# vvvwo/KSS-ICP

Hardware: AMD Instinct MI355X
Metric: icp_iterations_per_sec (higher is better)
Workload: dtype f32; 1 GPU; C2: one 100000x100000 uniform-sphere pair per GPU, 50 fixed ICP iterations + fitness pass per step (exact NN + cov reduce + host 3x3 SVD), R_z(10deg), jitter 1e-3; n_src=100000, n_tgt=100000, pairs_per_gpu=1, nn_engine=cell list + brute-force fallback, nn_arithmetic=reference (no fma)

## Files before the change

### kss-icp_amd/csrc/kss_engine.hip

```cpp
#pragma clang fp contract(off)

#include <emmintrin.h>
#include <limits>

#include "kss_ctx.hpp"
#include "kss_pair_device.hpp"

namespace kss {

static int restore_zero_at_rest(kss_ctx* c);

static int resident_rows_limit(kss_ctx* c) {
    if (c->cu_count <= 0) {
        hipDeviceProp_t prop;
        c->cu_count = hipGetDeviceProperties(&prop, c->device) == hipSuccess && prop.multiProcessorCount > 0 ? prop.multiProcessorCount : 1;
        (void)hipGetLastError();
    }
    return c->cu_count;
}

constexpr int PUB_PAIRS = 32;
static int ensure_pub(kss_ctx* c, int npairs = PUB_PAIRS);

struct PairGeom {
// ... 516 lines not shown
        hipDeviceProp_t prop;
        void* bar = nullptr;
        if (want_bar && hipGetDeviceProperties(&prop, c->device) == hipSuccess && prop.isLargeBar &&
            hipExtMallocWithFlags(&bar, 4096, hipDeviceMallocFinegrained) == hipSuccess && bar) {
            if (hipMemset(bar, 0, 4096) == hipSuccess && hipDeviceSynchronize() == hipSuccess) {
                c->gate_bar = (unsigned int*)bar;
                c->gated.supported = 1;
                return true;
            }
            hipFree(bar);
        }
        (void)hipGetLastError();
        void *x = nullptr, *xd = nullptr;
        if (ensure(c, c->g_gate, 256) == KSS_OK && hipMemsetAsync(c->g_gate.p, 0, 256, c->stream) == hipSuccess &&
            hipHostMalloc(&x, 2 * sizeof(PairState), hipHostMallocMapped) == hipSuccess && hipHostGetDevicePointer(&xd, x, 0) == hipSuccess) {
            std::memset(x, 0, 2 * sizeof(PairState));
            c->h_xf = (PairState*)x; c->h_xf_dev = (PairState*)xd;
            c->gated.supported = 1;
        } else {
            (void)hipGetLastError();
            if (x) hipHostFree(x);
        }
    }
    return c->gated.supported == 1;
}

static void gated_release(kss_ctx* c, const PairState& st, int skip) {
    if (c->gate_bar) {
        int words[16];
        std::memcpy(words, &st, sizeof st);
        words[14] = skip;
        unsigned int* slot = c->gate_bar + 32 * c->gated.slot;
        static const long torn_at = getenv("KSS_TEST_TORN_GATE") ? atol(getenv("KSS_TEST_TORN_GATE")) : -1;
        static long released = 0;
        const bool torn = ++released == torn_at;
        for (int pass = torn ? 0 : 1; pass < 2; ++pass) {
            for (int g = 0; g < 5; ++g) {
                const unsigned tag = (unsigned)c->gated.stamp + kss_mix3((unsigned)words[3 * g], (unsigned)words[3 * g + 1], (unsigned)words[3 * g + 2]);
                const int w1 = pass == 0 && g == 1 ? words[3 * g + 1] ^ 0x00010000 : words[3 * g + 1];
                const __m128i v = _mm_set_epi32((int)tag, words[3 * g + 2], w1, words[3 * g]);
                _mm_store_si128((__m128i*)(slot + 4 * g), v);
            }
            _mm_sfence();
            if (pass == 0) {
                const auto t0 = std::chrono::steady_clock::now();
                while (std::chrono::duration<double, std::micro>(std::chrono::steady_clock::now() - t0).count() < 200.0) __builtin_ia32_pause();
            }
        }
    } else {
        PairState* rec = &c->h_xf[c->gated.slot];
        for (int k = 0; k < 12; ++k) rec->m[k] = st.m[k];
        rec->active = st.active; rec->apply = st.apply; rec->pad[0] = skip;
        __atomic_store_n(&rec->pad[1], c->gated.stamp, __ATOMIC_RELEASE);
    }
    kss_ctx::Gated& G = c->gated;
    if (!skip && --G.steps_left > 0) {
        G.slot ^= 1;
        G.stamp += 1;
        G.seq += 1;
        const void* in = G.d_out; G.d_out = const_cast<void*>(G.d_in); G.d_in = in;
    } else {
        G.pending = false;
        G.steps_left = 0;
    }
}

static void gated_cancel(kss_ctx* c) {
    if (!c->gated.pending) return;
    PairState none;
    std::memset(&none, 0, sizeof none);
    gated_release(c, none, 1);
}

struct GatedGuard {
    kss_ctx* c;
    explicit GatedGuard(kss_ctx* c_) : c(c_) {}
    ~GatedGuard() { gated_cancel(c); c->gated.want_next = false; }
};

static float skin_setting() {
    static const float skin = getenv("KSS_SKIN") ? (float)atof(getenv("KSS_SKIN")) : 0.25f;
    return skin;
}
static int gate_polls_setting() {
    static const int gate_polls = getenv("KSS_GATE_POLLS") ? atoi(getenv("KSS_GATE_POLLS")) : (1 << 22);
    return gate_polls;
}

static PassArgs pass_args(kss_ctx* c, const IcpPlan& pl, const float4* d_in, float4* d_out, double max_d2,
                          int32_t* d_idx_out, float* d_d2_out) {
    PassArgs a;
    std::memset(&a, 0, sizeof a);
    a.src_in = d_in; a.src_out = d_out;
    a.cell_start = (const int32_t*)c->g_start.p + 1;
    a.sorted = (const float4*)c->g_sorted.p;
    a.tgt4 = (const float4*)c->tgt4.p;
    a.nn_win = (float4*)c->g_pos.p;
    a.nn_state = (float2*)c->g_nnst.p;
    a.skin = skin_setting();
    a.chain_len = 1;
    a.gate_polls = gate_polls_setting();
    a.chained = d_in != (const float4*)c->src0.p ? 1 : c->fit_last ? 2 : 0;
    a.src_last0 = (const float4*)c->cur[0].p; a.src_last1 = (const float4*)c->cur[1].p;
    a.keys = (unsigned long long*)c->keys.p;
    a.list = (int32_t*)c->g_list.p; a.list_count = (int32_t*)c->g_count.p;
    a.total_rows = pl.total_rows;
    a.use_prev = c->nn_have ? 1 : 0;
    a.max_d2 = max_d2;
    a.rows = (Granule*)c->partials.p;
    a.pub = c->h_seq_dev;
    a.idx_out = d_idx_out; a.d2_out = d_d2_out;
    {
        static const long torn_at = getenv("KSS_TEST_TORN_SLOT") ? atol(getenv("KSS_TEST_TORN_SLOT")) : -1;
        static long launches = 0;
        a.test_torn = torn_at > 0 && ++launches == torn_at ? 1 : 0;
    }
    if (pl.gridb) {
        a.pairs = (const GridPairDev*)c->g_pairs.p;
        a.row_pair = (const int32_t*)c->g_rowpair.p;
        a.defer_pairs = pl.npairs > resident_rows_limit(c) ? pl.npairs : 0;
    } else {
        a.pair0 = pl.gpairs[0];
    }
    return a;
}

struct GridPass {
    const IcpPlan& pl;
    bool fma, full;
    const float4* d_in; float4* d_out;
    double max_d2;
    int32_t* d_idx_out; float* d_d2_out;
    PassArgs a;
    int nblk;
    unsigned long long* stamps2 = nullptr;
    bool plain_args = false;
    unsigned long long want_seq = 0;
    bool via_gate = false;
};

static void grid_launch_plain(kss_ctx* c, GridPass& g) {
    ProfScope ps(c, KSS_K_GRID_NN);
    g.a.ps0 = ((const PairState*)c->h_state)[0];
    g.a.seq = ++c->seq;
    if (g.stamps2) g.a.stamps = g.stamps2 + (size_t)(g.a.seq & 1) * g.nblk * 16;
    launch_grid_pass(c->stream, g.fma, g.full, false, true, g.a);
    c->nn_have = true;
    g.want_seq = c->seq;
}

static void grid_release_or_launch(kss_ctx* c, GridPass& g) {
    kss_ctx::Gated& G = c->gated;
    if (G.pending && G.d_in == (const void*)g.d_in && G.d_out == (void*)g.d_out && G.fma == g.fma && G.full == g.full && G.max_d2 == g.max_d2 && g.plain_args) {
        g.want_seq = G.seq;
        c->seq = std::max(c->seq, G.seq);
        if (G.chain && c->prof > 0) c->prof_n[KSS_K_GRID_CHAIN_PASS] += 1;
        g.via_gate = true;
        static const long drop_at = getenv("KSS_TEST_DROP_GATE") ? atol(getenv("KSS_TEST_DROP_GATE")) : -1;
        static long releases = 0;
        if (++releases == drop_at) { G.pending = false; G.steps_left = 0; }
        else gated_release(c, ((const PairState*)c->h_state)[0], 0);
    } else {
        gated_cancel(c);
        grid_launch_plain(c, g);
    }
}

static void grid_enqueue_next(kss_ctx* c, const GridPass& g) {
    kss_ctx::Gated& G = c->gated;
    const bool next_sampled = c->prof == 1 || (c->prof > 1 && c->prof_tick[KSS_K_GRID_NN] % (unsigned)c->prof == 0);
    static const bool want_chain = getenv("KSS_CHAIN") == nullptr || atoi(getenv("KSS_CHAIN")) != 0;
    int len = 1;
    if (G.want_next && !G.pending && g.plain_args && gated_available(c) && want_chain && c->gate_bar &&
        (g.pl.total_rows <= resident_rows_limit(c) || g.pl.total_rows == 1))
        len = std::max(1, std::min(G.max_steps, 1 << 16));
    if (!(G.want_next && !G.pending && g.plain_args && gated_available(c) && (len > 1 || !next_sampled))) return;
    if (c->prof > 1 && len == 1) ++c->prof_tick[KSS_K_GRID_NN];
    float4* nxt_out = g.d_out == (float4*)c->cur[0].p ? (float4*)c->cur[1].p : (float4*)c->cur[0].p;
    G.slot ^= 1;
    G.stamp = (G.stamp + 1) & 0x7fffffff;
    if (G.stamp == 0 || G.stamp > 0x7fffffff - len - 1) G.stamp = 1;
    PassArgs n = pass_args(c, g.pl, g.d_out, nxt_out, g.max_d2, nullptr, nullptr);
// ... 1505 lines not shown
```

### kss-icp_amd/csrc/kss_grid.hip

```cpp
#pragma clang fp contract(off)

#include <hip/hip_runtime.h>

#include <cstring>

#include <rocprim/rocprim.hpp>

#include <cstdlib>

#include "kss_internal.hpp"
#include "kss_device.hpp"

namespace kss {

__global__ __launch_bounds__(256) void grid_count2_kernel(const float4* __restrict__ tgt, int nt, int nbt, const float4* __restrict__ src, int ns,
                                                          GridParams gp, int32_t* __restrict__ counts, int32_t* __restrict__ slot) {
    const bool is_src = (int)blockIdx.x >= nbt;
    const int i = ((int)blockIdx.x - (is_src ? nbt : 0)) * 256 + (int)threadIdx.x;
    if (i >= (is_src ? ns : nt)) return;
    const float4 p = is_src ? src[i] : tgt[i];
    const int cx = cell_coord(p.x, gp.ox, gp.inv_h, gp.gx), cy = cell_coord(p.y, gp.oy, gp.inv_h, gp.gy),
              cz = cell_coord(p.z, gp.oz, gp.inv_h, gp.gz);
    slot[(is_src ? nt : 0) + i] = atomicAdd(&counts[(is_src ? gp.gx * gp.gy * gp.gz : 0) + (cz * gp.gy + cy) * gp.gx + cx], 1);
}
// ... 537 lines not shown
                    const int x0 = max(cx - r, 0), x1 = min(cx + r, gp.gx - 1);
                    for (int t = 0; t < wd * wd; ++t) {
                        const int dz = t / wd - r, dy = t % wd - r;
                        const int z = cz + dz, y = cy + dy;
                        if (z < 0 || z >= gp.gz || y < 0 || y >= gp.gy) continue;
                        const int row = (z * gp.gy + y) * gp.gx;
                        if (dz == -r || dz == r || dy == -r || dy == r) {
                            scan_range<FMA>(sorted, cs[row + x0], cs[row + x1 + 1], wx, wy, wz, wkey, wpos);
                        } else {
                            if (cx - r >= 0) scan_range<FMA>(sorted, cs[row + cx - r], cs[row + cx - r + 1], wx, wy, wz, wkey, wpos);
                            if (cx + r < gp.gx) scan_range<FMA>(sorted, cs[row + cx + r], cs[row + cx + r + 1], wx, wy, wz, wkey, wpos);
                        }
                    }
                }
                const float best = __uint_as_float((unsigned)(wkey >> 32));
                float b = __builtin_inff();
                if (cx - r > 0) b = fminf(b, wx - (gp.ox + (float)(cx - r) * gp.h));
                if (cx + r < gp.gx - 1) b = fminf(b, (gp.ox + (float)(cx + r + 1) * gp.h) - wx);
                if (cy - r > 0) b = fminf(b, wy - (gp.oy + (float)(cy - r) * gp.h));
                if (cy + r < gp.gy - 1) b = fminf(b, (gp.oy + (float)(cy + r + 1) * gp.h) - wy);
                if (cz - r > 0) b = fminf(b, wz - (gp.oz + (float)(cz - r) * gp.h));
                if (cz + r < gp.gz - 1) b = fminf(b, (gp.oz + (float)(cz + r + 1) * gp.h) - wz);
                const float bs = b - gp.eps;
                if (b == __builtin_inff()) done = true;
                else if (bs > 0.f && best < bs * bs * 0.999999f) { done = true; face2 = bs * bs; }
                if (done) { rfin = r; break; }
            }
            if (done && rfin == 1 && wkey != ~0ull)
                bnew = fminf(__builtin_amdgcn_sqrtf(fminf(fminf(m2, wrho), face2) * 0.99999f) * 0.999999f, 1e30f);
        }
        if constexpr (BATCH) {
            if (__builtin_amdgcn_ballot_w64(!done) != 0ull) {
                const float4* __restrict__ tp = a.tgt4 + pr.tgt_base;
                for (int j = 0; j < pr.tgt_n; ++j) {
                    const float4 q = tp[j];
                    const float dx = wx - q.x, dy = wy - q.y, dz = wz - q.z;
                    float d;
                    if constexpr (FMA) d = __builtin_fmaf(dx, dx, __builtin_fmaf(dy, dy, dz * dz));
                    else d = (dx * dx + dy * dy) + dz * dz;
                    const unsigned long long kk = ((unsigned long long)__float_as_uint(d) << 32) | (unsigned long long)(unsigned)j;
                    if (!done && kk < wkey) { wkey = kk; wpos = -1; }
                }
                wfell = !done;
                done = true;
            }
        }
        if (wk && sub == 0) {
            bool whave = false;
            float4 ww = make_float4(0.f, 0.f, 0.f, 0.f);
            const int io = pr.src_base + (w - pr.row_base) * PASS_BS + owner;
            if (done) {
                whave = wkey != ~0ull;
                if (whave) ww = wpos >= 0 ? sorted[wpos] : wpos == -2 ? a.nn_win[io] : a.tgt4[pr.tgt_base + (int)(unsigned)(wkey & 0xffffffffull)];
            } else {
                a.keys[io] = ~0ull;
                const int ls = atomicAdd(a.list_count, 1);
                a.list[ls] = io;
                wfell = true;
            }
            a.nn_win[io] = make_float4(ww.x, ww.y, ww.z, __uint_as_float(whave ? (unsigned)wkey : ~0u));
            a.nn_state[io] = make_float2(wfell ? 0.f : bnew, 0.f);
            s_ent[WK_X][owner] = __float_as_uint(ww.x); s_ent[WK_Y][owner] = __float_as_uint(ww.y); s_ent[WK_Z][owner] = __float_as_uint(ww.z);
            s_ent[WK_IDX][owner] = (unsigned)wkey; s_ent[WK_D2][owner] = (unsigned)(wkey >> 32);
            s_ent[WK_FL][owner] = (whave ? 1u : 0u) | (wfell ? 2u : 0u);
            s_ent[WK_R][owner] = __float_as_uint(wfell ? 0.f : bnew);
        }
        KSS_STAMP(8);
        if (a.stamps) {
            int evs = evl, mx = evl;
#pragma unroll
            for (int m = 32; m > 0; m >>= 1) { evs += __shfl_xor(evs, m, 64); mx = max(mx, __shfl_xor(mx, m, 64)); }
            if (lane == 0) {
                atomicAdd(&a.stamps[(size_t)blockIdx.x * 16 + 10], (unsigned long long)evs);
                atomicAdd(&a.stamps[(size_t)blockIdx.x * 16 + 11], (unsigned long long)(((mx + 7) / 8) * 8 * 64));
            }
        }
    }
#undef KSS_STAMP
}

#ifndef KSS_SINGLE_WAVES
#define KSS_SINGLE_WAVES 1
#endif
template <bool FMA, bool FULL, bool SEARCH, bool CHAIN, bool FIRST = false>
__global__ __launch_bounds__(PASS_BS, KSS_SINGLE_WAVES) void grid_pass_kernel(const PassArgs a) {
    static_assert(!CHAIN || SEARCH, "chained launches: search passes");
    static_assert(!FIRST || (SEARCH && !CHAIN), "the first pass: a plain search launch");
#define KSS_STAMP(k) do { if (a.stamps && threadIdx.x == 0) a.stamps[(size_t)blockIdx.x * 16 + (k)] = __builtin_amdgcn_s_memrealtime(); } while (0)
    KSS_STAMP(0);
    constexpr int BS = PASS_BS;
    const int per_xcd = (int)gridDim.x / 8;
    const int w = ((int)blockIdx.x % 8) * per_xcd + (int)blockIdx.x / 8;
    if (w >= a.total_rows) return;
    const GridPairDev pr = a.pair0;
    PairState ps = a.ps0;
    const GridParams& gp = pr.gp;
    const int32_t* __restrict__ cs = a.cell_start + pr.cell_base;
    const float4* __restrict__ sorted = a.sorted;
    constexpr int WQ = FIRST ? BS : 256;
    __shared__ int2 rowq[9][WQ];
    __shared__ double shw[BS / 64][NSUMS];
    __shared__ int s_last;
    __shared__ int sh_ps[16];
    __shared__ int s_nwalk;
    __shared__ unsigned s_ent[7][BS];
    __shared__ unsigned short s_wl[BS];
    enum { WK_X, WK_Y, WK_Z, WK_IDX, WK_D2, WK_R, WK_POS, WK_FL = WK_POS, WK_COLS };
    static_assert(sizeof(PairState) == 64, "the gated launch reads the transform record as 16 dwords");
    double (*shf)[NSUMS] = reinterpret_cast<double (*)[NSUMS]>(&rowq[0][0]);
    static_assert(sizeof(double) * PASS_FG * NSUMS <= sizeof(int2) * 9 * WQ, "shf must fit inside rowq");

    const int local = (w - pr.row_base) * BS + (int)threadIdx.x;
    const bool valid = local < pr.src_n;
    const int i = pr.src_base + local;
    const int lane = threadIdx.x & 63, wave = threadIdx.x >> 6;
    bool have = false, fell_back = false;
    float qx = 0.f, qy = 0.f, qz = 0.f, d2 = 0.f;
    float4 win = make_float4(0.f, 0.f, 0.f, 0.f);
    float4 p = make_float4(0.f, 0.f, 0.f, 0.f), prevp = make_float4(0.f, 0.f, 0.f, __uint_as_float(~0u));
    float2 st = make_float2(0.f, 0.f);
    if (valid) {
        p = SEARCH ? a.src_in[i] : a.src_out[i];
        if (!SEARCH || a.use_prev) { prevp = a.nn_win[i]; st = a.nn_state[i]; }
    }
    for (int step = 0;; ++step) {
    const bool last_step = !CHAIN || step + 1 >= a.chain_len;
    const unsigned long long seq_k = a.seq + (unsigned long long)step;
    const int gate_k = a.gate_seq != 0 ? a.gate_seq + step : 0;
    unsigned int* const gate_ptr = a.gate_dev + 32 * ((a.gate_slot + step) & 1);
    float4* const src_out_k = (step & 1) ? a.src_alt : a.src_out;
    const bool last_known = a.chained == 2 && ps.pad[0] > 0;
    const bool chained_k = step > 0 || a.chained == 1 || last_known;
    const bool has_prev = __float_as_uint(prevp.w) != ~0u;
    if constexpr (SEARCH) {
        __syncthreads();
        if (threadIdx.x == 0) s_nwalk = 0;
        __syncthreads();
    }
    KSS_STAMP(13);
    if constexpr (SEARCH) {
        if (gate_k != 0) {
            typedef unsigned int u32x4 __attribute__((ext_vector_type(4)));
            if (a.state && w == 0 && threadIdx.x < 16) {
                const int* w32 = reinterpret_cast<const int*>(a.state);
                int v = 0, n = 0;
                bool ok = true;
                for (;;) {
                    v = __hip_atomic_load(w32 + threadIdx.x, __ATOMIC_RELAXED, __HIP_MEMORY_SCOPE_SYSTEM);
                    if (__shfl(v, 15, 64) == gate_k) break;
                    __builtin_amdgcn_s_sleep(1);
                    if (++n > a.gate_polls / 2) { ok = false; break; }
                }
                if (ok) {
                    const int g = threadIdx.x;
                    const int w0 = __shfl(v, min(3 * g, 15), 64), w1 = __shfl(v, min(3 * g + 1, 15), 64), w2 = __shfl(v, min(3 * g + 2, 15), 64);
                    if (g < 5) {
                        u32x4 o;
                        o.x = (unsigned)w0; o.y = (unsigned)w1; o.z = (unsigned)w2; o.w = (unsigned)gate_k + kss_mix3(o.x, o.y, o.z);
                        unsigned int* dst = gate_ptr + 4 * g;
                        asm volatile("global_store_dwordx4 %0, %1, off sc1" ::"v"(dst), "v"(o) : "memory");
                    }
                }
            }
            if (threadIdx.x < 8) {
                const unsigned int* src = gate_ptr + 4 * min((int)threadIdx.x, 4);
                u32x4 v;
                int n = 0;
                bool ok = true;
                for (;;) {
                    asm volatile("global_load_dwordx4 %0, %1, off sc0 sc1\n\ts_waitcnt vmcnt(0)" : "=&v"(v) : "v"(src) : "memory");
                    if (__builtin_amdgcn_ballot_w64(v.w - kss_mix3(v.x, v.y, v.z) == (unsigned)gate_k) == 0xffull) break;
                    __builtin_amdgcn_s_sleep(1);
                    if (++n > a.gate_polls) { ok = false; break; }
                }
                if (threadIdx.x < 5) { sh_ps[3 * threadIdx.x] = (int)v.x; sh_ps[3 * threadIdx.x + 1] = (int)v.y; sh_ps[3 * threadIdx.x + 2] = (int)v.z; }
                if (threadIdx.x == 0) { sh_ps[15] = gate_k; s_last = ok ? 1 : 0; }
            }
            __syncthreads();
            if (!s_last) return;
            int* d32 = reinterpret_cast<int*>(&ps);
#pragma unroll
            for (int k = 0; k < 16; ++k) d32[k] = sh_ps[k];
            if (ps.pad[0] != 0) return;
            __syncthreads();
            KSS_STAMP(9);
        }
    }
    unsigned long long key = ~0ull;
    float pold_x = p.x, pold_y = p.y, pold_z = p.z;
    if (SEARCH && last_known && valid) {
        const float4 pl = (ps.pad[0] == 1 ? a.src_last0 : a.src_last1)[i];
        pold_x = pl.x; pold_y = pl.y; pold_z = pl.z;
    }
    if (valid) {
        if constexpr (SEARCH) {
            if (ps.apply) {
                const float x = p.x, y = p.y, z = p.z;
                p.x = ((ps.m[0] * x + ps.m[1] * y) + ps.m[2] * z) + ps.m[3];
                p.y = ((ps.m[4] * x + ps.m[5] * y) + ps.m[6] * z) + ps.m[7];
                p.z = ((ps.m[8] * x + ps.m[9] * y) + ps.m[10] * z) + ps.m[11];
            }
            src_out_k[i] = p;
        }
        qx = p.x; qy = p.y; qz = p.z;
        const bool qok = (qx - qx) == 0.f && (qy - qy) == 0.f && (qz - qz) == 0.f;
        if constexpr (!SEARCH) {
            if (has_prev) {
                win = prevp;
                key = point_key<FMA>(win, qx, qy, qz);
            } else if (qok) {
                key = a.keys[i];
                if (key != ~0ull) win = a.tgt4[pr.tgt_base + (int)(unsigned)(key & 0xffffffffull)];
            }
            have = key != ~0ull;
        }
    }
    if constexpr (SEARCH) {
        bool walker = false;
        float acc_keep = 0.f;
        {
            const bool qok = valid && (qx - qx) == 0.f && (qy - qy) == 0.f && (qz - qz) == 0.f;
            const SkipOut so = skip_test<FMA>(qok, qx, qy, qz, pold_x, pold_y, pold_z, prevp, st, chained_k, a.skin, gp.h);
            walker = so.walker;
            key = so.key;
            acc_keep = so.acc;
            unsigned fl = 0u;
            if (qok && !walker) {
                fl = 1u;
                a.nn_state[i] = make_float2(st.x, so.acc);
            } else if (valid && !qok) {
                a.nn_win[i] = make_float4(0.f, 0.f, 0.f, __uint_as_float(~0u));
                a.nn_state[i] = make_float2(0.f, 0.f);
            }
            const float4 c4 = walker ? make_float4(qx, qy, qz, 0.f) : prevp;
            s_ent[WK_X][threadIdx.x] = __float_as_uint(c4.x); s_ent[WK_Y][threadIdx.x] = __float_as_uint(c4.y); s_ent[WK_Z][threadIdx.x] = __float_as_uint(c4.z);
            s_ent[WK_IDX][threadIdx.x] = (unsigned)key; s_ent[WK_D2][threadIdx.x] = (unsigned)(key >> 32);
            s_ent[WK_POS][threadIdx.x] = walker ? (unsigned)so.kpos : fl;
            s_ent[WK_R][threadIdx.x] = __float_as_uint(so.rho);
        }
        const unsigned long long wm = __builtin_amdgcn_ballot_w64(walker);
        if (wm != 0ull) {
            int base = 0;
            if (lane == 0) base = atomicAdd(&s_nwalk, (int)__builtin_popcountll(wm));
            base = __builtin_amdgcn_readfirstlane(base);
            if (walker) s_wl[base + (int)__builtin_amdgcn_mbcnt_hi((unsigned)(wm >> 32), __builtin_amdgcn_mbcnt_lo((unsigned)wm, 0u))] = (unsigned short)threadIdx.x;
        }
        KSS_STAMP(14);
        __syncthreads();
        const int nwalk = s_nwalk;
        if (a.stamps && threadIdx.x == 0) a.stamps[(size_t)blockIdx.x * 16 + 12] = (unsigned long long)nwalk;
        serve_walkers<FMA, false, WQ, BS, 8, FIRST>(a, pr, cs, sorted, w, nwalk, rowq, s_ent, s_wl);
        KSS_STAMP(15);
        __syncthreads();
        {
            const unsigned fl = s_ent[WK_FL][threadIdx.x];
            have = (fl & 1u) != 0u; fell_back = (fl & 2u) != 0u;
            win = make_float4(__uint_as_float(s_ent[WK_X][threadIdx.x]), __uint_as_float(s_ent[WK_Y][threadIdx.x]), __uint_as_float(s_ent[WK_Z][threadIdx.x]), 0.f);
            key = ((unsigned long long)s_ent[WK_D2][threadIdx.x] << 32) | (unsigned long long)s_ent[WK_IDX][threadIdx.x];
            if (CHAIN && !last_step) {
                if (walker) {
                    prevp = make_float4(win.x, win.y, win.z, __uint_as_float(have ? (unsigned)key : ~0u));
                    st = make_float2(__uint_as_float(s_ent[WK_R][threadIdx.x]), 0.f);
                } else if (have) {
                    st.y = acc_keep;
                } else {
                    prevp.w = __uint_as_float(~0u);
                    st = make_float2(0.f, 0.f);
                }
            }
        }
    }
    if (valid && have) {
        d2 = __uint_as_float((unsigned)(key >> 32));
        const int oi = __float_as_int(p.w);
        if (a.idx_out) a.idx_out[oi] = (int)(unsigned)(key & 0xffffffffull);
        if (a.d2_out) a.d2_out[oi] = d2;
    }
    KSS_STAMP(1);

    const double d2d = have ? (double)d2 : 0.0;
    const bool kept = have && !(d2d > a.max_d2);
    wave_row<FULL>(have, kept, fell_back, qx, qy, qz, win, d2d, shw[wave]);
    __syncthreads();
    double r = 0.0;
    if (threadIdx.x < NSUMS)
#pragma unroll
        for (int ww = 0; ww < BS / 64; ++ww) r += shw[ww][threadIdx.x];
    KSS_STAMP(2);

    double v = 0.0 + r;
    if (pr.n_rows > 1) {
        Granule* const rows = a.rows + (int64_t)pr.row_base * NSUMS;
        if (threadIdx.x < NSUMS) row_put(rows + (int64_t)(w - pr.row_base) * NSUMS, threadIdx.x, r, seq_k);
        KSS_STAMP(3);
        if (w != pr.row_base || a.defer_pairs) {
            if (last_step) return;
            continue;
        }
        if (!rows_total<PASS_FG>(rows, pr.n_rows, seq_k, 1 << 20, shf, &s_last, v)) return;
    }
    if (threadIdx.x < NSUMS) {
        if (!FULL && (threadIdx.x == 17 || threadIdx.x == 18)) v = 0.0;
        const int64_t slot = threadIdx.x;
        if (a.test_torn && threadIdx.x == 5) {
            pub_put(a.pub, slot, v, seq_k, 0x00100000u);
            asm volatile("s_waitcnt vmcnt(0)" ::: "memory");
            for (int k = 0; k < 400; ++k) __builtin_amdgcn_s_sleep(64);
        }
        pub_put(a.pub, slot, v, seq_k);
        KSS_STAMP(4);
    }
    if (last_step) break;
    }
#undef KSS_STAMP
}

#ifndef KSS_BATCH2_WAVES
#define KSS_BATCH2_WAVES 5
#endif
template <bool FMA, bool FULL, int WQ>
__global__ __launch_bounds__(256, KSS_BATCH2_WAVES) void gridb_pass_kernel(const PassArgs a) {
#define KSS_STAMP(k) do { if (a.stamps && threadIdx.x == 0) a.stamps[(size_t)blockIdx.x * 16 + (k)] = __builtin_amdgcn_s_memrealtime(); } while (0)
    KSS_STAMP(0);
    constexpr int BS = PASS_BS, NT = 256, SPL = BS / NT;
    static_assert(SPL == 2 && WQ <= NT, "two sources per lane");
    const int per_xcd = (int)gridDim.x / 8;
    const int w = ((int)blockIdx.x % 8) * per_xcd + (int)blockIdx.x / 8;
    if (w >= a.total_rows) return;
    const int pi = a.row_pair[w];
    const GridPairDev pr = a.pairs[pi];
    const PairState ps = a.state[pi];
    if (!ps.active) return;
    const GridParams& gp = pr.gp;
    const int32_t* __restrict__ cs = a.cell_start + pr.cell_base;
    const float4* __restrict__ sorted = a.sorted;
    __shared__ int2 rowq[9][WQ];
    __shared__ double shw[BS / 64][NSUMS];
    __shared__ int s_last;
    __shared__ int s_nwalk;
    __shared__ unsigned s_ent[7][BS];
    __shared__ unsigned short s_wl[BS];
    enum { WK_X, WK_Y, WK_Z, WK_IDX, WK_D2, WK_R, WK_POS, WK_FL = WK_POS, WK_COLS };
    constexpr int SHF_ROWS = (int)(sizeof(int2) * 9 * WQ / (sizeof(double) * NSUMS));
    static_assert(SHF_ROWS >= PASS_FG, "shf must fit inside rowq");
    double (*shf)[NSUMS] = reinterpret_cast<double (*)[NSUMS]>(&rowq[0][0]);
    const int lane = threadIdx.x & 63, wave = threadIdx.x >> 6;

    bool valid[SPL];
    int idx[SPL];
    float4 p[SPL], prevp[SPL];
    float2 st[SPL];
#pragma unroll
    for (int k = 0; k < SPL; ++k) {
        const int slot = k * NT + (int)threadIdx.x;
        const int local = (w - pr.row_base) * BS + slot;
        valid[k] = local < pr.src_n;
        idx[k] = pr.src_base + local;
        p[k] = make_float4(0.f, 0.f, 0.f, 0.f);
        prevp[k] = make_float4(0.f, 0.f, 0.f, __uint_as_float(~0u));
        st[k] = make_float2(0.f, 0.f);
        if (valid[k]) {
            p[k] = a.src_in[idx[k]];
            if (a.use_prev) { prevp[k] = a.nn_win[idx[k]]; st[k] = a.nn_state[idx[k]]; }
        }
    }
    if (threadIdx.x == 0) s_nwalk = 0;
    __syncthreads();
    KSS_STAMP(13);
    const bool last_known = a.chained == 2 && ps.pad[0] > 0;
    const bool chained_k = a.chained == 1 || last_known;
    bool walker[SPL];
#pragma unroll
    for (int k = 0; k < SPL; ++k) {
        const int slot = k * NT + (int)threadIdx.x;
        const int i = idx[k];
        float pold_x = p[k].x, pold_y = p[k].y, pold_z = p[k].z;
        if (last_known && valid[k]) {
            const float4 pl = (ps.pad[0] == 1 ? a.src_last0 : a.src_last1)[i];
            pold_x = pl.x; pold_y = pl.y; pold_z = pl.z;
// ... 323 lines not shown
#pragma unroll
        for (int u = 0; u < GB_U; ++u) p[u] = sp[min(k0 + u * GB_THREADS, pr.src_n - 1)];
#pragma unroll
        for (int u = 0; u < GB_U; ++u) {
            const int k = k0 + u * GB_THREADS;
            if (k < pr.src_n) {
                const int pos = cnt.add1(cell_of(p[u]));
                p[u].w = __int_as_float(pr.src_base + k);
                tmp[pos] = p[u];
            }
        }
    }
    __syncthreads();
    float4* out = src_out + pr.src_base;
    for (int j0 = tid; j0 < pr.src_n; j0 += GB_THREADS * GB_U) {
        float4 p[GB_U];
#pragma unroll
        for (int u = 0; u < GB_U; ++u) p[u] = tmp[min(j0 + u * GB_THREADS, pr.src_n - 1)];
#pragma unroll
        for (int u = 0; u < GB_U; ++u) {
            if (j0 + u * GB_THREADS >= pr.src_n) continue;
            const int c = cell_of(p[u]);
            const int lo = c > 0 ? cnt.get(c - 1) : 0, hi = cnt.get(c);
            const int me = __float_as_int(p[u].w);
            int rank = 0;
            for (int k = lo; k < hi; ++k) rank += __float_as_int(tmp[k].w) < me ? 1 : 0;
            out[lo + rank] = p[u];
        }
    }
}

bool launch_gridb_build_lds(hipStream_t st, const float4* d_tgt4, float4* d_src, float4* d_tmp, const GridPairDev* d_pairs, int npairs,
                            int32_t* d_cell_start, float4* d_sorted, int max_cells, bool half) {
    const size_t bytes = half ? (size_t)((max_cells + 1) / 2) * 4 : (size_t)max_cells * 4;
    {
        const int most = GB_MAX_CELLS * 4;
        const void* fn = half ? reinterpret_cast<const void*>(&gridb_build_pair_kernel<true>) : reinterpret_cast<const void*>(&gridb_build_pair_kernel<false>);
        if (hipFuncSetAttribute(fn, hipFuncAttributeMaxDynamicSharedMemorySize, most) != hipSuccess) { (void)hipGetLastError(); return false; }
    }
    if (half)
        hipLaunchKernelGGL(gridb_build_pair_kernel<true>, dim3(npairs), dim3(GB_THREADS), bytes, st, d_tgt4, (const float4*)d_src, d_tmp, d_src, d_pairs,
                           d_cell_start, d_sorted);
    else
        hipLaunchKernelGGL(gridb_build_pair_kernel<false>, dim3(npairs), dim3(GB_THREADS), bytes, st, d_tgt4, (const float4*)d_src, d_tmp, d_src, d_pairs,
                           d_cell_start, d_sorted);
    return true;
}

__global__ __launch_bounds__(256) void grid_stats_kernel(const float4* __restrict__ src, int ns, GridParams gp,
                                                         const int32_t* __restrict__ cell_start, unsigned long long* __restrict__ out) {
    const int i = blockIdx.x * blockDim.x + threadIdx.x;
    unsigned long long ev = 0, occ = 0;
    if (i < ns) {
        const float4 p = src[i];
        const int cx = cell_coord(p.x, gp.ox, gp.inv_h, gp.gx), cy = cell_coord(p.y, gp.oy, gp.inv_h, gp.gy),
                  cz = cell_coord(p.z, gp.oz, gp.inv_h, gp.gz);
        const int x0 = max(cx - 1, 0), x1 = min(cx + 1, gp.gx - 1);
        for (int t = 0; t < 9; ++t) {
            const int z = cz + t / 3 - 1, y = cy + t % 3 - 1;
            if (z < 0 || z >= gp.gz || y < 0 || y >= gp.gy) continue;
            const int row = (z * gp.gy + y) * gp.gx;
            ev += (unsigned long long)(cell_start[row + x1 + 1] - cell_start[row + x0]);
        }
    }
    const int ncells = gp.gx * gp.gy * gp.gz;
    for (int c = blockIdx.x * blockDim.x + threadIdx.x; c < ncells; c += gridDim.x * blockDim.x)
        occ += cell_start[c + 1] > cell_start[c] ? 1 : 0;
    atomicAdd(&out[0], ev);
    atomicAdd(&out[1], occ);
}

void launch_grid_stats(hipStream_t st, const float4* d_src, int ns, const GridParams& gp, const int32_t* d_cell_start,
                       unsigned long long* d_out) {
    hipLaunchKernelGGL(grid_stats_kernel, dim3((ns + 255) / 256), dim3(256), 0, st, d_src, ns, gp, d_cell_start, d_out);
}

int grid_pass_blocks(int total_rows) { return (total_rows + 7) / 8 * 8; }

void launch_grid_pass(hipStream_t st, bool fma, bool full, bool batch, bool search, const PassArgs& a) {
    if (a.total_rows <= 0) return;
    const dim3 grid(grid_pass_blocks(a.total_rows)), block(PASS_BS);
    static const bool first_pass = getenv("KSS_FIRST_PASS") == nullptr || atoi(getenv("KSS_FIRST_PASS")) != 0;
#define KSS_PASS(F, U, S) hipLaunchKernelGGL((grid_pass_kernel<F, U, S, false>), grid, block, 0, st, a)
#define KSS_CHAIN(F, U) hipLaunchKernelGGL((grid_pass_kernel<F, U, true, true>), grid, block, 0, st, a)
    if (!search) {
        if (fma) KSS_PASS(true, true, false); else KSS_PASS(false, true, false);
    } else if (batch) {
        const dim3 block2(256);
#define KSS_PASSB(F, U, Q) hipLaunchKernelGGL((gridb_pass_kernel<F, U, Q>), grid, block2, 0, st, a)
        if (!a.use_prev) {
            if (fma) { if (full) KSS_PASSB(true, true, 256); else KSS_PASSB(true, false, 256); }
            else     { if (full) KSS_PASSB(false, true, 256); else KSS_PASSB(false, false, 256); }
        } else {
            if (fma) { if (full) KSS_PASSB(true, true, 128); else KSS_PASSB(true, false, 128); }
            else     { if (full) KSS_PASSB(false, true, 128); else KSS_PASSB(false, false, 128); }
        }
#undef KSS_PASSB
        if (a.defer_pairs) hipLaunchKernelGGL(gridb_finalize_kernel, dim3(a.defer_pairs), dim3(256), 0, st, a, full ? 1 : 0);
    } else if (a.chain_len > 1) {
        if (fma) { if (full) KSS_CHAIN(true, true); else KSS_CHAIN(true, false); }
        else     { if (full) KSS_CHAIN(false, true); else KSS_CHAIN(false, false); }
    } else if (first_pass && !a.use_prev) {
#define KSS_FIRST(F, U) hipLaunchKernelGGL((grid_pass_kernel<F, U, true, false, true>), grid, block, 0, st, a)
        if (fma) { if (full) KSS_FIRST(true, true); else KSS_FIRST(true, false); }
        else     { if (full) KSS_FIRST(false, true); else KSS_FIRST(false, false); }
#undef KSS_FIRST
    } else {
        if (fma) { if (full) KSS_PASS(true, true, true); else KSS_PASS(true, false, true); }
        else     { if (full) KSS_PASS(false, true, true); else KSS_PASS(false, false, true); }
    }
#undef KSS_PASS
#undef KSS_CHAIN
}

}
```

### kss-icp_amd/csrc/kss_internal.hpp

```cpp
#pragma once
#include <hip/hip_runtime.h>

#include <algorithm>
#include <cfloat>
#include <cmath>
#include <cstdint>
#include <functional>
#include <string>
#include <vector>

#include "../../include/kssicp.h"
#include "kss_host_math.hpp"

namespace kss {

struct alignas(16) PairState {
    float m[12];
    int32_t active;
    int32_t apply;
    int32_t pad[2];
};

struct alignas(16) NNWork {
    int32_t pair;
// ... 7 lines not shown
};

struct alignas(16) RedWork {
    int32_t pair;
    int32_t src_begin;
    int32_t src_count;
    int32_t key_begin;
    int32_t key_stride;
    int32_t n_split;
    int32_t tgt_pair_base;
    int32_t partial_index;
};

struct PairRed {
    int32_t first;
    int32_t count;
};

__host__ __device__ inline unsigned kss_mix3(unsigned a, unsigned b, unsigned c) {
    unsigned h = (a + 0x9E3779B1u) * 0x85EBCA77u;
    h ^= h >> 15;
    h = (h ^ (b + 0x7F4A7C15u)) * 0xC2B2AE3Du;
    h ^= h >> 13;
    h = (h ^ (c + 0x165667B1u)) * 0x27D4EB2Fu;
    h ^= h >> 16;
    return h;
}

struct GridParams {
    float ox, oy, oz;
    float h, inv_h;
    float eps;
    int32_t gx, gy, gz;
    int32_t rcap;
};

struct alignas(16) GridPairDev {
    GridParams gp;
    int32_t cell_base;
    int32_t tgt_base, tgt_n;
    int32_t src_base, src_n;
    int32_t tgt_pad;
    int32_t row_base, n_rows;
    int32_t sorted_base;
};

struct PackSeg {
    int64_t in_off;
    int64_t out_base;
    int64_t n;
};

struct alignas(16) Granule { unsigned long long bits, seq; };

struct PassArgs {
    const float4* src_in; float4* src_out;
    const int32_t* cell_start;
    const float4* sorted;
    const float4* tgt4;
    float4* nn_win;
    float2* nn_state;
    int32_t chained;
    const float4* src_last0; const float4* src_last1;
    float skin;
    unsigned long long* keys;
    int32_t* list; int32_t* list_count;
    const GridPairDev* pairs;
    const int32_t* row_pair;
    const PairState* state;
    GridPairDev pair0; PairState ps0;
    int32_t total_rows, use_prev;
    int32_t gate_polls;
    int32_t chain_len, gate_slot;
    float4* src_alt;
    int32_t gate_seq;
    int32_t defer_pairs;
    unsigned int* gate_dev;
    double max_d2;
    Granule* rows;
    unsigned long long* pub; unsigned long long seq;
    int32_t* idx_out; float* d2_out;
    unsigned long long* stamps;
    int32_t test_torn;
};

constexpr int RES_THREADS = 1024;
constexpr int RES_SMAX = 10;
constexpr int RES_NQ = 640;
constexpr int RES_QW = 4;
constexpr int RES_G = 4;
constexpr int RES_LDS_MAX = 160 * 1024 - 256;
constexpr unsigned RES_STAMP_ANY = 4095u;
__device__ __forceinline__ void res_store_exit_flag(unsigned long long* flags, int pair, unsigned tag, unsigned note = 0u) {
    typedef unsigned int u32x4 __attribute__((ext_vector_type(4)));
    u32x4 o;
    o.x = tag; o.y = (unsigned)pair; o.z = note; o.w = kss_mix3(o.x, o.y, o.z);
    unsigned long long* dst = flags + 2 * (int64_t)pair;
    asm volatile("global_store_dwordx4 %0, %1, off sc0 sc1" ::"v"(dst), "v"(o) : "memory");
}
struct ResArgs {
    const GridPairDev* pairs;
    const int32_t* cell_start;
    const float4* sorted;
    const float4* src0;
    unsigned int* gate;
    unsigned long long* pub;
    unsigned long long seq0;
    unsigned int stamp0;
    double max_d2;
    float skin;
    int32_t gate_polls, max_passes, full_always;
    int32_t ntc, tabc;
    int32_t* idx_out; float* d2_out;
    unsigned long long* exit_flags;
    unsigned int exit_tag;
    const int32_t* perm;
    int32_t first_pass, split_at;
    float4* st_pos; unsigned int* st_wc;
    unsigned long long* stamps;
};
size_t resident_lds_bytes(int ntc, int tabc);
int launch_resident(hipStream_t st, bool fma, int npairs, const ResArgs& a, std::string& err);

struct OctBox {
    double min[3], max[3];
    double res;
    int32_t depth;
};

constexpr int NN_TILE = 256;
constexpr int NN_SUB = 32;
constexpr int NN_THREADS = 256;

inline void oct_first_point(OctBox& b, const float* p) {
    const float minValue = FLT_EPSILON;
    for (int k = 0; k < 3; ++k) { b.min[k] = p[k] - b.res / 2; b.max[k] = p[k] + b.res / 2; }
    unsigned maxv = 2;
    for (int k = 0; k < 3; ++k) maxv = std::max(maxv, (unsigned)std::ceil((b.max[k] - b.min[k] - minValue) / b.res));
    b.depth = (int)std::ceil(std::log2((double)maxv) - minValue);
    const double side = (double)(1u << b.depth) * b.res;
    for (int k = 0; k < 3; ++k) {
        const double over = (side - (b.max[k] - b.min[k])) / 2.0;
        if (over > minValue) { b.min[k] -= over; b.max[k] += over; }
    }
}
inline bool oct_adopt(OctBox& b, const float* p) {
    const float minValue = FLT_EPSILON;
    for (;;) {
        bool up[3], any = false;
        for (int k = 0; k < 3; ++k) { up[k] = p[k] >= b.max[k]; any = any || up[k] || p[k] < b.min[k]; }
        if (!any) return true;
        if (b.depth >= 21) return false;
        double side = (double)(1u << b.depth) * b.res;
        for (int k = 0; k < 3; ++k) if (!up[k]) b.min[k] -= side;
        ++b.depth;
        side = (double)(1u << b.depth) * b.res - minValue;
        for (int k = 0; k < 3; ++k) b.max[k] = b.min[k] + side;
    }
}

void launch_pack_f3_to_f4(hipStream_t st, const float* d_in, int64_t n, float4* d_out, int64_t n_pad, bool sentinel);
void launch_pack_f64_to_f4(hipStream_t st, const double* d_in, int64_t n, float4* d_out, int64_t n_pad, bool sentinel);
void launch_empty(hipStream_t st);
int pack_pair_bbox_rows(int64_t nt_pad);
void launch_pack_pair(hipStream_t st, int dtype, const void* d_tgt, int64_t nt, float4* d_tgt_out, int64_t nt_pad, float* d_bbox_partial,
                      const void* d_src, int64_t ns, float4* d_src_out, unsigned int* d_box_host, unsigned box_tag);
// ... 262 lines not shown
```

Before: 82820 iterations/s.

## Cache per-point near-neighbor candidate lists in LDS for chained ICP search passes

Adds a per-block LDS cache holding the three nearest target candidates per source point, along with a safety radius, for the chained search kernel. A certified lower bound accounts for accumulated motion, and when it still holds, a point takes its nearest neighbour from the cached candidates instead of walking the cell list. Between chained steps, points whose margin is shrinking get their lists refreshed cooperatively, 16 lanes per point. The aim is to cut repeated grid walks across ICP iterations, at the cost of extra LDS (dynamic shared memory), extra block syncs, and refresh work that could lower occupancy or add overhead.

```diff
diff --git a/kss-icp_amd/csrc/kss_engine.hip b/kss-icp_amd/csrc/kss_engine.hip
--- a/kss-icp_amd/csrc/kss_engine.hip
+++ b/kss-icp_amd/csrc/kss_engine.hip
@@ -622,6 +622,13 @@
     static const float skin = getenv("KSS_SKIN") ? (float)atof(getenv("KSS_SKIN")) : 0.25f;
     return skin;
 }
+#ifndef KSS_NEAR_K
+#define KSS_NEAR_K 10
+#endif
+static int near_lists_setting() {
+    static const int k = getenv("KSS_NEAR_LISTS") ? std::max(0, std::min(atoi(getenv("KSS_NEAR_LISTS")), 1000)) : KSS_NEAR_K;
+    return k;
+}
 static int gate_polls_setting() {
     static const int gate_polls = getenv("KSS_GATE_POLLS") ? atoi(getenv("KSS_GATE_POLLS")) : (1 << 22);
     return gate_polls;
@@ -638,6 +645,7 @@
     a.nn_win = (float4*)c->g_pos.p;
     a.nn_state = (float2*)c->g_nnst.p;
     a.skin = skin_setting();
+    a.near_lists = near_lists_setting();
     a.chain_len = 1;
     a.gate_polls = gate_polls_setting();
     a.chained = d_in != (const float4*)c->src0.p ? 1 : c->fit_last ? 2 : 0;
diff --git a/kss-icp_amd/csrc/kss_grid.hip b/kss-icp_amd/csrc/kss_grid.hip
--- a/kss-icp_amd/csrc/kss_grid.hip
+++ b/kss-icp_amd/csrc/kss_grid.hip
@@ -643,6 +643,105 @@
 #ifndef KSS_SINGLE_WAVES
 #define KSS_SINGLE_WAVES 1
 #endif
+constexpr int NEAR_N = 3;
+constexpr int NEAR_MAXB = 32;
+constexpr int NEAR_U = 32;
+struct NearPts { float4 pt[NEAR_N][PASS_BS]; };
+template <bool ON>
+struct NearLds {
+    float lb[PASS_BS], mv[PASS_BS];
+    unsigned short bl[NEAR_MAXB];
+    int cnt[PASS_BS / 64];
+};
+template <>
+struct NearLds<false> {};
+
+template <bool FMA>
+__device__ __forceinline__ void near_refresh(const PassArgs& a, const GridParams& gp, const int32_t* __restrict__ cs, const float4* __restrict__ sorted,
+                                             NearLds<true>& nl, NearPts* npts, unsigned (*s_ent)[PASS_BS], bool chosen, float qx, float qy, float qz, float dw2) {
+    const int tid = (int)threadIdx.x, lane = tid & 63, wave = tid >> 6;
+    const unsigned long long cm = __builtin_amdgcn_ballot_w64(chosen);
+    if (lane == 0) nl.cnt[wave] = (int)__builtin_popcountll(cm);
+    if (chosen) {
+        s_ent[0][tid] = __float_as_uint(qx); s_ent[1][tid] = __float_as_uint(qy); s_ent[2][tid] = __float_as_uint(qz);
+        s_ent[3][tid] = __float_as_uint(dw2);
+    }
+    __syncthreads();
+    int base = 0, nb = 0;
+#pragma unroll
+    for (int ww = 0; ww < PASS_BS / 64; ++ww) { const int c = nl.cnt[ww]; base += ww < wave ? c : 0; nb += c; }
+    if (chosen) {
+        const int slot = base + (int)__builtin_amdgcn_mbcnt_hi((unsigned)(cm >> 32), __builtin_amdgcn_mbcnt_lo((unsigned)cm, 0u));
+        if (slot < NEAR_MAXB) nl.bl[slot] = (unsigned short)tid;
+    }
+    nb = min(nb, NEAR_MAXB);
+    __syncthreads();
+    if ((tid & ~63) >= nb * 16) return;
+    const int g = tid >> 4, sub = tid & 15;
+    const bool wk = g < nb;
+    const int owner = wk ? (int)nl.bl[g] : 0;
+    const float wx = __uint_as_float(s_ent[0][owner]), wy = __uint_as_float(s_ent[1][owner]), wz = __uint_as_float(s_ent[2][owner]);
+    const float wd2 = __uint_as_float(s_ent[3][owner]);
+    const int cx = cell_coord(wx, gp.ox, gp.inv_h, gp.gx), cy = cell_coord(wy, gp.oy, gp.inv_h, gp.gy), cz = cell_coord(wz, gp.oz, gp.inv_h, gp.gz);
+    const float grown = __builtin_amdgcn_sqrtf(wd2) + fmaxf(a.skin, 0.f) * gp.h;
+    const float rho = fmaxf(wd2, grown * grown);
+    int lo, hi;
+    row_range(gp, cs, wx, wy, wz, cx, cy, cz, rho, wk && sub < 9 ? sub : -1, lo, hi);
+    const int n = hi - lo;
+    unsigned keys[NEAR_U];
+#pragma unroll
+    for (int h = 0; h < NEAR_U; h += 16) {
+        float4 pt[16];
+#pragma unroll
+        for (int j = 0; j < 16; ++j) pt[j] = sorted[n > 0 ? min(lo + h + j, hi - 1) : 0];
+#pragma unroll
+        for (int j = 0; j < 16; ++j)
+            keys[h + j] = h + j < n ? ((unsigned)(point_key<FMA>(pt[j], wx, wy, wz) >> 32) & ~0x1ffu) | (unsigned)(sub << 5) | (unsigned)(h + j) : ~0u;
+    }
+    float b = __builtin_inff();
+    if (cx - 1 > 0) b = fminf(b, wx - (gp.ox + (float)(cx - 1) * gp.h));
+    if (cx + 1 < gp.gx - 1) b = fminf(b, (gp.ox + (float)(cx + 2) * gp.h) - wx);
+    if (cy - 1 > 0) b = fminf(b, wy - (gp.oy + (float)(cy - 1) * gp.h));
+    if (cy + 1 < gp.gy - 1) b = fminf(b, (gp.oy + (float)(cy + 2) * gp.h) - wy);
+    if (cz - 1 > 0) b = fminf(b, wz - (gp.oz + (float)(cz - 1) * gp.h));
+    if (cz + 1 < gp.gz - 1) b = fminf(b, (gp.oz + (float)(cz + 2) * gp.h) - wz);
+    const float bs = b - gp.eps;
+    const float face2 = b == __builtin_inff() ? __builtin_inff() : bs * bs;
+    const unsigned over = (unsigned)(__builtin_amdgcn_ballot_w64(n > NEAR_U) >> (lane & 48)) & 0xffffu;
+    const bool ok = wk && over == 0u && (b == __builtin_inff() || (bs > 0.f && wd2 < bs * bs * 0.999999f));
+    auto x1 = [](int v) { return __builtin_amdgcn_update_dpp(0, v, 0xb1, 0xf, 0xf, false); };
+    auto x2 = [](int v) { return __builtin_amdgcn_update_dpp(0, v, 0x4e, 0xf, 0xf, false); };
+    auto x4 = [](int v) { const int r = __builtin_amdgcn_update_dpp(v, v, 0x104, 0xf, 0x5, false); return __builtin_amdgcn_update_dpp(r, v, 0x114, 0xf, 0xa, false); };
+    auto x8 = [](int v) { return __builtin_amdgcn_update_dpp(0, v, 0x128, 0xf, 0xf, false); };
+    unsigned last = 0u;
+    float mk = __builtin_inff();
+    int mine[NEAR_N];
+#pragma unroll
+    for (int r = 0; r <= NEAR_N; ++r) {
+        unsigned gm = ~0u;
+#pragma unroll
+        for (int j = 0; j < NEAR_U; ++j) gm = min(gm, r == 0 || keys[j] > last ? keys[j] : ~0u);
+        gm = min(gm, (unsigned)x1((int)gm)); gm = min(gm, (unsigned)x2((int)gm)); gm = min(gm, (unsigned)x4((int)gm)); gm = min(gm, (unsigned)x8((int)gm));
+        if (r < NEAR_N) {
+            mine[r] = ok && gm != ~0u && (int)((gm >> 5) & 15u) == sub ? lo + (int)(gm & 31u) : -1;
+            if (ok && gm == ~0u && sub == 0) npts->pt[r][owner] = make_float4(0.f, 0.f, 0.f, __uint_as_float(~0u));
+        } else if (gm != ~0u) {
+            mk = __uint_as_float(gm & ~0x1ffu);
+        }
+        last = gm;
+    }
+    {
+        float4 tk[NEAR_N];
+#pragma unroll
+        for (int r = 0; r < NEAR_N; ++r) tk[r] = sorted[max(mine[r], 0)];
+#pragma unroll
+        for (int r = 0; r < NEAR_N; ++r) if (mine[r] >= 0) npts->pt[r][owner] = tk[r];
+    }
+    if (ok && sub == 0) {
+        nl.lb[owner] = fminf(__builtin_amdgcn_sqrtf(fminf(fminf(mk, rho), face2) * 0.99999f) * 0.999999f, 1e30f);
+        nl.mv[owner] = 0.f;
+    }
+}
 template <bool FMA, bool FULL, bool SEARCH, bool CHAIN, bool FIRST = false>
 __global__ __launch_bounds__(PASS_BS, KSS_SINGLE_WAVES) void grid_pass_kernel(const PassArgs a) {
     static_assert(!CHAIN || SEARCH, "chained launches: search passes");
@@ -666,6 +765,9 @@
     __shared__ int s_nwalk;
     __shared__ unsigned s_ent[7][BS];
     __shared__ unsigned short s_wl[BS];
+    __shared__ NearLds<CHAIN> nl;
+    extern __shared__ float4 near_dyn[];
+    NearPts* const npts = reinterpret_cast<NearPts*>(near_dyn);
     enum { WK_X, WK_Y, WK_Z, WK_IDX, WK_D2, WK_R, WK_POS, WK_FL = WK_POS, WK_COLS };
     static_assert(sizeof(PairState) == 64, "the gated launch reads the transform record as 16 dwords");
     double (*shf)[NSUMS] = reinterpret_cast<double (*)[NSUMS]>(&rowq[0][0]);
@@ -683,6 +785,10 @@
     if (valid) {
         p = SEARCH ? a.src_in[i] : a.src_out[i];
         if (!SEARCH || a.use_prev) { prevp = a.nn_win[i]; st = a.nn_state[i]; }
+    }
+    if constexpr (CHAIN) {
+        nl.lb[threadIdx.x] = 0.f;
+        nl.mv[threadIdx.x] = 0.f;
     }
     for (int step = 0;; ++step) {
     const bool last_step = !CHAIN || step + 1 >= a.chain_len;
@@ -785,10 +891,44 @@
             walker = so.walker;
             key = so.key;
             acc_keep = so.acc;
+            if constexpr (CHAIN) {
+                const float lb = nl.lb[threadIdx.x];
+                if (qok && lb > 0.f && a.near_lists != 0) {
+                    const float mx = qx - pold_x, my = qy - pold_y, mz = qz - pold_z;
+                    const float mvl = (nl.mv[threadIdx.x] + __builtin_amdgcn_sqrtf((mx * mx + my * my) + mz * mz)) * 1.00001f;
+                    nl.mv[threadIdx.x] = mvl;
+                    if (walker && has_prev) {
+                        unsigned long long bk = ~0ull;
+                        float4 bp = prevp;
+                        float n1 = __builtin_inff(), n2 = __builtin_inff();
+#pragma unroll
+                        for (int j = 0; j < NEAR_N; ++j) {
+                            const float4 pj = npts->pt[j][threadIdx.x];
+                            const bool used = __float_as_uint(pj.w) != ~0u;
+                            const unsigned long long kk = used ? point_key<FMA>(pj, qx, qy, qz) : ~0ull;
+                            const float dd = used ? __uint_as_float((unsigned)(kk >> 32)) : __builtin_inff();
+                            n2 = __builtin_amdgcn_fmed3f(n1, n2, dd);
+                            n1 = fminf(n1, dd);
+                            if (kk < bk) { bk = kk; bp = pj; }
+                        }
+                        const float room = lb - mvl;
+                        if (bk != ~0ull && room > 1e-7f && __uint_as_float((unsigned)(bk >> 32)) < (room * room) * 0.99999f) {
+                            walker = false;
+                            key = bk;
+                            prevp = bp;
+                            st.x = n2 < __builtin_inff() ? fminf(__builtin_amdgcn_sqrtf(fminf(n2, room * room) * 0.99999f) * 0.999999f, 1e30f) : 0.f;
+                            acc_keep = 0.f;
+                            a.nn_win[i] = prevp;
+                        }
+                    }
+                } else if (valid && !qok) {
+                    nl.lb[threadIdx.x] = 0.f;
+                }
+            }
             unsigned fl = 0u;
             if (qok && !walker) {
                 fl = 1u;
-                a.nn_state[i] = make_float2(st.x, so.acc);
+                a.nn_state[i] = make_float2(st.x, acc_keep);
             } else if (valid && !qok) {
                 a.nn_win[i] = make_float4(0.f, 0.f, 0.f, __uint_as_float(~0u));
                 a.nn_state[i] = make_float2(0.f, 0.f);
@@ -856,6 +996,21 @@
         KSS_STAMP(3);
         if (w != pr.row_base || a.defer_pairs) {
             if (last_step) return;
+            if constexpr (CHAIN) {
+                if (a.near_lists != 0) {
+                    bool chosen = false;
+                    if (valid && have && !fell_back && chained_k) {
+                        const float mx = qx - pold_x, my = qy - pold_y, mz = qz - pold_z;
+                        const float budget = (float)a.near_lists * __builtin_amdgcn_sqrtf((mx * mx + my * my) + mz * mz);
+                        const float dw = __builtin_amdgcn_sqrtf(d2);
+                        if ((st.x - st.y) - dw < budget) {
+                            const float lb = nl.lb[threadIdx.x];
+                            chosen = !(lb > 0.f) || (lb - nl.mv[threadIdx.x]) - dw < budget;
+                        }
+                    }
+                    near_refresh<FMA>(a, gp, cs, sorted, nl, npts, s_ent, chosen, qx, qy, qz, d2);
+                }
+            }
             continue;
         }
         if (!rows_total<PASS_FG>(rows, pr.n_rows, seq_k, 1 << 20, shf, &s_last, v)) return;
@@ -1345,7 +1500,7 @@
     const dim3 grid(grid_pass_blocks(a.total_rows)), block(PASS_BS);
     static const bool first_pass = getenv("KSS_FIRST_PASS") == nullptr || atoi(getenv("KSS_FIRST_PASS")) != 0;
 #define KSS_PASS(F, U, S) hipLaunchKernelGGL((grid_pass_kernel<F, U, S, false>), grid, block, 0, st, a)
-#define KSS_CHAIN(F, U) hipLaunchKernelGGL((grid_pass_kernel<F, U, true, true>), grid, block, 0, st, a)
+#define KSS_CHAIN(F, U) hipLaunchKernelGGL((grid_pass_kernel<F, U, true, true>), grid, block, sizeof(NearPts), st, a)
     if (!search) {
         if (fma) KSS_PASS(true, true, false); else KSS_PASS(false, true, false);
     } else if (batch) {
diff --git a/kss-icp_amd/csrc/kss_internal.hpp b/kss-icp_amd/csrc/kss_internal.hpp
--- a/kss-icp_amd/csrc/kss_internal.hpp
+++ b/kss-icp_amd/csrc/kss_internal.hpp
@@ -113,6 +113,7 @@
     int32_t* idx_out; float* d2_out;
     unsigned long long* stamps;
     int32_t test_torn;
+    int32_t near_lists;
 };
 
 constexpr int RES_THREADS = 1024;
```

Result: slower. 80870 iterations/s (-2.4%).
